# andi611/ZeroSpeech-TTS-without-T

Hardware: AMD Instinct MI355X
Metric: mel-frames/sec (train_ae, seg_len=128, enc_size=1024) (higher is better)
Workload: dtype bf16; 1 GPU; train_ae english hps seg_len=128 enc_size=1024 emb_size=1024 n_speakers=102 F=513, batch=256/GPU, dropout+Gumbel on, fwd+bwd+clip+Adam; global_batch=256, parallelism=dp1

## Files before the change

include/zs_amd.h:

```cpp
#ifndef ZS_AMD_H
#define ZS_AMD_H
#include <stddef.h>
#include <stdint.h>

#ifdef __cplusplus
extern "C" {
#endif

#define ZS_ABI_VERSION 1

enum { ZS_F32 = 0, ZS_BF16 = 1 };
enum { ZS_OK = 0, ZS_EINVAL = -1, ZS_ELAUNCH = -2, ZS_EWORKSPACE = -3 };
enum { ZS_PAD_ZERO = 0, ZS_PAD_REFLECT = 1 };
enum { ZS_ACT_NONE = 0, ZS_ACT_LRELU = 1, ZS_ACT_SIGMOID = 2, ZS_ACT_TANH = 3 };
enum { ZS_STORE_ROWS = 0, ZS_STORE_SPLIT2 = 1 };
enum { ZS_RES_NONE = 0, ZS_RES_IDENTITY = 1, ZS_RES_AVGPOOL2 = 2, ZS_RES_UPSAMPLE2 = 3 };

int zs_abi_version(void);
const char* zs_last_error(void);
int zs_set_option(const char* key, int value);

typedef struct {
  int32_t dtype;
  const void* A; int64_t lda; int64_t a_batch_stride;
// ... 80 lines not shown
  const void* x; int64_t ldx;
  void* out; int64_t ldo;
  void* out2; int64_t ldo2; const float* vec2; int64_t vec2_ld; int32_t vec2_cols; const int64_t* idx;
  float* mean; float* rstd;
  int32_t B, T, C; float eps;
  float drop_p; uint64_t seed; uint32_t stream_id; const uint8_t* mask; int64_t mask_ld;
  int32_t res_mode; const void* res; int64_t ldres; int32_t T_res; int32_t res_pad_mode;
  const uint64_t* seed_ptr;
  const int32_t* lengths; const int32_t* res_lengths;
  int32_t stats_given;
} ZsInstNormFwd;
int zs_instnorm_fwd(const ZsInstNormFwd* p, void* stream);

typedef struct {
  int32_t dtype;
  const void* dout; int64_t ldd;
  const void* x; int64_t ldx;
  const float* mean; const float* rstd;
  void* dz; int64_t ldz;
  int32_t B, T, C;
  float drop_p; uint64_t seed; uint32_t stream_id; const uint8_t* mask; int64_t mask_ld;
  float slope;
  const uint64_t* seed_ptr;
} ZsInstNormBwd;
int zs_instnorm_bwd(const ZsInstNormBwd* p, void* stream);

typedef struct {
  int32_t dtype;
  const void* gp; int64_t ldg; int32_t pad_left, pad_right, pad_mode;
  int32_t B, T, C;
  float* emb_sum; int64_t emb_ld; int32_t emb_cols;
  int32_t res_mode; const void* res; int64_t ldres;
  const void* dact_src; int64_t dact_ld; float slope;
  void* out; int64_t ldo; int32_t unshuffle;
} ZsGradCombine;
int zs_grad_combine(const ZsGradCombine* p, void* stream);
int zs_norm_decomposition(int32_t kernel, int32_t dtype, int32_t T, int32_t C);

typedef struct {
  const float* emb_sum; int64_t emb_ld; const int64_t* idx; int32_t B;
  float* demb; int64_t demb_ld; int32_t n_rows, C; int32_t accumulate;
} ZsEmbScatter;
int zs_emb_scatter(const ZsEmbScatter* p, void* stream);

typedef struct {
  int32_t dtype;
  const void* logits; int64_t ld; int32_t logits_f32;
  const float* noise; int32_t noise_kind; uint64_t seed;
  int64_t rows; int32_t E; float tau;
  void* bits; int64_t ld_bits; int32_t bits_fill_cols;
  float* bits_f32;
  float* y0;
  const uint64_t* seed_ptr;
} ZsMbvFwd;
int zs_mbv_fwd(const ZsMbvFwd* p, void* stream);
typedef struct {
  int32_t dtype;
  const void* dbits; int64_t ld_dbits;
  const float* y0; int64_t rows; int32_t E; float tau;
  void* dlogits; int64_t ld; int32_t fill_cols;
} ZsMbvBwd;
int zs_mbv_bwd(const ZsMbvBwd* p, void* stream);

enum { ZS_ENC_ONE_HOT = 0, ZS_ENC_BINARY = 1, ZS_ENC_CONTINUES = 2 };
typedef struct {
  int32_t dtype; int32_t mode;
// ... 295 lines not shown
```

zerospeech-tts-without-t_amd/_lib.py:

```python
import ctypes
import os
import re

_PKG = os.path.dirname(os.path.abspath(__file__))
_ROOT = os.path.dirname(_PKG)
HEADER = os.path.join(_ROOT, 'include', 'zs_amd.h')
_SAN = os.environ.get('ZS_SANITIZE', '').strip()
LIB_PATH = os.environ.get('ZS_LIB_PATH') or os.path.join(_PKG, 'libzs_amd.%s.so' % _SAN if _SAN else 'libzs_amd.so')

_CTYPES = {
    'int32_t': ctypes.c_int32, 'int64_t': ctypes.c_int64, 'uint32_t': ctypes.c_uint32, 'uint64_t': ctypes.c_uint64,
    'float': ctypes.c_float, 'double': ctypes.c_double, 'size_t': ctypes.c_size_t, 'int': ctypes.c_int,
}


def _strip_comments(text):
    return re.sub(r'/\*.*?\*/', ' ', text, flags=re.S)


def parse_header(path=HEADER):
    text = _strip_comments(open(path).read())
    structs = {}
    for body, name in re.findall(r'typedef\s+struct\s*\{(.*?)\}\s*(\w+)\s*;', text, flags=re.S):
        fields = []
# ... 142 lines not shown
        self._outer = (_PACK, _VEC)
        _PACK, _VEC = [], []
        return self

    def __exit__(self, et, ev, tb):
        global _PACK, _VEC
        jobs, vjobs = _PACK, _VEC
        _PACK, _VEC = self._outer
        if et is None and jobs:
            S = STRUCTS['ZsPackWeight']
            arr = (S * len(jobs))(*jobs)
            fn = lib().zs_pack_weight_batch
            fn.argtypes = [ctypes.c_void_p, ctypes.c_int32, ctypes.c_int32, ctypes.c_void_p]
            check(fn(ctypes.addressof(arr), len(jobs), 0, self.stream), 'zs_pack_weight_batch')
        if et is None and vjobs:
            S = STRUCTS['ZsVecCopy']
            arr = (S * len(vjobs))(*vjobs)
            fn = lib().zs_copy_vec_batch
            fn.argtypes = [ctypes.c_void_p, ctypes.c_int32, ctypes.c_void_p]
            check(fn(ctypes.addressof(arr), len(vjobs), self.stream), 'zs_copy_vec_batch')
        return False


def call(fname, sname, stream, **kw):
    try:
        s = STRUCTS[sname](**{k: v for k, v in kw.items() if v is not None})
    except TypeError as e:
        raise KeyError('%s: %s' % (sname, e))
    if _PACK is not None and fname == 'zs_pack_weight':
        _PACK.append(s)
        return s
    fn = _FN.get(fname)
    if fn is None:
        fn = getattr(lib(), fname)
        fn.argtypes = [ctypes.c_void_p, ctypes.c_void_p]
        _FN[fname] = fn
    rc = fn(ctypes.addressof(s), stream)
    if rc != 0:
        check(rc, fname)
    return s
```

zerospeech-tts-without-t_amd/csrc/zs_elem.hip:

```cpp
#include <string.h>

#include "zs_common.h"

namespace {

constexpr int NTE = 256;

template <typename T> __device__ __forceinline__ float ldT(const void* p, int64_t i) { return Elem<T>::ld((const T*)p + i); }
template <typename T> __device__ __forceinline__ void stT(void* p, int64_t i, float v) { Elem<T>::st((T*)p + i, v); }

template <typename T>
__device__ __forceinline__ void pack_weight_body(const ZsPackWeight& p, int64_t first, int64_t step) {
  const int64_t total = (int64_t)p.n_rows * p.n_cols;
  for (int64_t i = first; i < total; i += step) {
    const int row = (int)(i / p.n_cols);
    const int k = (int)(i - (int64_t)row * p.n_cols);
    const int tap = k / p.inner_pad, inner = k - tap * p.inner_pad;
    int n, ci;
    if (p.transpose == 0) { n = row; ci = inner; } else { n = inner; ci = row; }
    float v = 0.f;
    if (n < p.Cout && ci < p.Cin && tap < p.taps) {
      const int half = p.Cout >> 1;
      const int co = p.row_perm ? p.row_perm[n] : (p.co_split2 ? (n < half ? 2 * n : 2 * (n - half) + 1) : n);
      v = p.W[(int64_t)co * p.so + (int64_t)ci * p.si + (int64_t)tap * p.sj];
// ... 177 lines not shown
__global__ __launch_bounds__(128) void emb_scatter_kernel(const ZsEmbScatter p) {
  __shared__ int list[128];
  __shared__ int wcount[2];
  const int tid = threadIdx.x, lane = tid & 63, wave = tid >> 6;
  const int c = blockIdx.x * 128 + tid;
  const int r = blockIdx.y;
  float s = 0.f;
  for (int b0 = 0; b0 < p.B; b0 += 128) {
    const int b = b0 + tid;
    const bool hit = b < p.B && p.idx[b] == (int64_t)r;
    const unsigned long long m = __ballot(hit);
    if (lane == 0) wcount[wave] = __popcll(m);
    __syncthreads();
    const int n0 = wcount[0], n = n0 + wcount[1];
    if (hit) list[(wave ? n0 : 0) + __popcll(m & ((1ull << lane) - 1ull))] = b;
    __syncthreads();
    if (c < p.C)
      for (int i = 0; i < n; ++i) s += p.emb_sum[(int64_t)list[i] * p.emb_ld + c];
    __syncthreads();
  }
  if (c >= p.C) return;
  float* d = p.demb + (int64_t)r * p.demb_ld + c;
  *d = p.accumulate ? (*d + s) : s;
}

template <typename T>
__global__ void mbv_fwd_kernel(const ZsMbvFwd p) {
  const int64_t total = p.rows * p.bits_fill_cols;
  const uint64_t seed = p.seed + (p.seed_ptr ? *p.seed_ptr : 0ull);
  for (int64_t i = (int64_t)blockIdx.x * blockDim.x + threadIdx.x; i < total; i += (int64_t)gridDim.x * blockDim.x) {
    const int64_t r = i / p.bits_fill_cols;
    const int e = (int)(i - r * p.bits_fill_cols);
    float bit = 0.f;
    if (e < p.E) {
      float l0, l1;
      if (p.logits_f32) { l0 = ((const float*)p.logits)[r * p.ld + 2 * e]; l1 = ((const float*)p.logits)[r * p.ld + 2 * e + 1]; }
      else { l0 = ldT<T>(p.logits, r * p.ld + 2 * e); l1 = ldT<T>(p.logits, r * p.ld + 2 * e + 1); }
      const int64_t ni = (r * p.E + e) * 2;
      float g0, g1;
      if (p.noise_kind == 0) { g0 = p.noise[ni]; g1 = p.noise[ni + 1]; }
      else {
        float u0, u1;
        if (p.noise_kind == 1) { u0 = p.noise[ni]; u1 = p.noise[ni + 1]; }
        else { u0 = zs_uniform(seed, 0x6d627600u, (uint64_t)ni); u1 = zs_uniform(seed, 0x6d627600u, (uint64_t)ni + 1); }
        g0 = -logf(-logf(u0 + 1e-20f) + 1e-20f);
        g1 = -logf(-logf(u1 + 1e-20f) + 1e-20f);
// ... 319 lines not shown
  ZS_DISPATCH(p->dtype, add_rowvec_kernel, dim3(nblocks((int64_t)p->B * p->T * p->fill_cols, 4096)), dim3(NTE), stream, *p);
  return zs_check_launch("zs_add_rowvec");
}

extern "C" int zs_rows_reverse(const ZsRowsReverse* p, void* stream) {
  ZS_REQUIRE(p && p->x && p->B > 0 && p->T > 0 && p->cols > 0 && p->col0 >= 0 && p->ld >= (int64_t)p->col0 + p->cols, "zs_rows_reverse: bad args");
  ZS_REQUIRE(p->dtype == ZS_F32 || p->dtype == ZS_BF16, "zs_rows_reverse: bad dtype");
  const int es = p->dtype == ZS_F32 ? 4 : 2;
  ZS_REQUIRE((p->cols * es) % 4 == 0 && (p->col0 * es) % 4 == 0 && (p->ld * es) % 4 == 0 && (((uintptr_t)p->x) & 3) == 0,
             "zs_rows_reverse: the column block must be made of whole 4-byte words");
  if (p->T < 2) return ZS_OK;
  const int words = p->cols * es / 4;
  hipLaunchKernelGGL(rows_reverse_kernel, dim3(nblocks((int64_t)p->B * (p->T >> 1) * words, 4096)), dim3(NTE), 0, (hipStream_t)stream, *p, words,
                     (int64_t)p->ld * es, (int64_t)p->col0 * es);
  return zs_check_launch("zs_rows_reverse");
}

extern "C" int zs_emb_scatter(const ZsEmbScatter* p, void* stream) {
  ZS_REQUIRE(p && p->emb_sum && p->idx && p->demb && p->B > 0 && p->n_rows > 0 && p->C > 0, "zs_emb_scatter: bad args");
  hipLaunchKernelGGL(emb_scatter_kernel, dim3((p->C + 127) / 128, p->n_rows), dim3(128), 0, (hipStream_t)stream, *p);
  return zs_check_launch("zs_emb_scatter");
}

extern "C" int zs_mbv_fwd(const ZsMbvFwd* p, void* stream) {
  ZS_REQUIRE(p && p->logits && p->rows > 0 && p->E > 0 && p->tau > 0.f, "zs_mbv_fwd: bad args");
  ZS_REQUIRE(p->dtype == ZS_F32 || p->dtype == ZS_BF16, "zs_mbv_fwd: bad dtype");
  ZS_REQUIRE(p->noise_kind == 2 || p->noise, "zs_mbv_fwd: noise missing");
  ZS_REQUIRE(p->bits || p->bits_f32, "zs_mbv_fwd: no output");
  ZsMbvFwd q = *p;
  if (!q.bits || q.bits_fill_cols < q.E) q.bits_fill_cols = q.E;
  ZS_DISPATCH(p->dtype, mbv_fwd_kernel, dim3(nblocks(q.rows * q.bits_fill_cols)), dim3(NTE), stream, q);
  return zs_check_launch("zs_mbv_fwd");
}

extern "C" int zs_mbv_bwd(const ZsMbvBwd* p, void* stream) {
  ZS_REQUIRE(p && p->dbits && p->y0 && p->dlogits && p->rows > 0 && p->E > 0 && p->fill_cols >= 2 * p->E && p->fill_cols % 2 == 0,
             "zs_mbv_bwd: bad args");
  ZS_REQUIRE(p->dtype == ZS_F32 || p->dtype == ZS_BF16, "zs_mbv_bwd: bad dtype");
  ZS_DISPATCH(p->dtype, mbv_bwd_kernel, dim3(nblocks(p->rows * (p->fill_cols / 2))), dim3(NTE), stream, *p);
  return zs_check_launch("zs_mbv_bwd");
}

extern "C" int zs_l1_loss(const ZsL1Loss* p, void* stream) {
  ZS_REQUIRE(p && p->x_dec && p->x && p->partial && p->loss_out && p->rows > 0 && p->F > 0, "zs_l1_loss: bad args");
  ZS_REQUIRE(p->dtype == ZS_F32 || p->dtype == ZS_BF16, "zs_l1_loss: bad dtype");
  ZsL1Loss q = *p;
// ... 48 lines not shown
```

zerospeech-tts-without-t_amd/csrc/zs_norm.hip:

```cpp
#include <stdlib.h>

#include "zs_common.h"

namespace {

constexpr int RPT = 8;
struct Narrow { static constexpr int NTN = 256, CHUNK = 64, RG = 32; };
struct Wide8 { static constexpr int NTN = 256, CHUNK = 256, RG = 8; };
constexpr int RGN = 32;

template <typename S>
__device__ __forceinline__ void colreduce(const float (&pv)[RGN / S::RG][8], float (&out)[8], float* red, float* tot, int cg, int rg, int tid) {
  constexpr int CHUNK = S::CHUNK, RG = S::RG, NP = RGN / RG;
#pragma unroll
  for (int j = 0; j < NP; ++j)
#pragma unroll
    for (int k = 0; k < 8; ++k) red[(rg + RG * j) * CHUNK + cg * 8 + k] = pv[j][k];
  __syncthreads();
  for (int c = tid; c < CHUNK; c += S::NTN) {
    float s = 0.f;
#pragma unroll 8
    for (int r = 0; r < RGN; ++r) s += red[r * CHUNK + c];
    tot[c] = s;
  }
// ... 171 lines not shown
    if (cvalid && t < p.T) {
      const int64_t row = (int64_t)b * p.T + t;
      g[i].ld((const T*)p.dout + row * p.ldd + c0);
      xv[i].ld((const T*)p.x + row * p.ldx + c0);
    }
  }
#pragma unroll
  for (int i = 0; i < RPT; ++i) {
    const int t = rg + RG * i;
    if (cvalid && t < p.T) {
      const int64_t row = (int64_t)b * p.T + t;
      float gf[8], xf[8];
      g[i].cvt(gf); xv[i].cvt(xf);
#pragma unroll
      for (int k = 0; k < 8; ++k) {
        gf[k] *= keep_scale(p.mask, p.mask_ld, p.drop_p, seed, p.stream_id, row, c0 + k, p.C, inv_keep);
        const float xh = (xf[k] - mean[k]) * rstd[k];
        pg[i % NP][k] += gf[k]; pgx[i % NP][k] += gf[k] * xh;
      }
    }
  }
  colreduce<S>(pg, sg, red, tot, cg, rg, tid);
  colreduce<S>(pgx, sgx, red, tot, cg, rg, tid);
  if (!cvalid) return;
  const float invT = 1.f / (float)p.T;
#pragma unroll
  for (int i = 0; i < RPT; ++i) {
    const int t = rg + RG * i;
    if (t >= p.T) continue;
    const int64_t row = (int64_t)b * p.T + t;
    float o[8], gf[8], xf[8];
    g[i].cvt(gf); xv[i].cvt(xf);
#pragma unroll
    for (int k = 0; k < 8; ++k) {
      gf[k] *= keep_scale(p.mask, p.mask_ld, p.drop_p, seed, p.stream_id, row, c0 + k, p.C, inv_keep);
      const float xh = (xf[k] - mean[k]) * rstd[k];
      const float dx = rstd[k] * (gf[k] - sg[k] * invT - xh * (sgx[k] * invT));
      o[k] = dx * dlrelu_f(xf[k], p.slope);
    }
    store8<T>((T*)p.dz + row * p.ldz + c0, o);
  }
}

template <typename T, typename S>
__global__ __launch_bounds__(S::NTN) void grad_combine_kernel(const ZsGradCombine p) {
  constexpr int CHUNK = S::CHUNK, RG = S::RG, CGN = S::CHUNK / 8, NP = RGN / RG;
  __shared__ float red[RGN * CHUNK];
  __shared__ float tot[CHUNK];
  const int tid = threadIdx.x, cg = tid % CGN, rg = tid / CGN;
  const int b = blockIdx.y, c0 = blockIdx.x * CHUNK + cg * 8;
  const bool cvalid = c0 < p.C;
  const int Tp = p.T + p.pad_left + p.pad_right;
  const T* gp = (const T*)p.gp;
  float v[RPT][8];
  float ps[NP][8], s[8];
#pragma unroll
  for (int j = 0; j < NP; ++j)
#pragma unroll
    for (int k = 0; k < 8; ++k) ps[j][k] = 0.f;
#pragma unroll
  for (int i = 0; i < RPT; ++i) {
    const int t = rg + RG * i;
#pragma unroll
// ... 140 lines not shown
```

zerospeech-tts-without-t_amd/engine.py:

```python
import functools
import os
import torch

from . import _lib as L
from .layers import (Act, ConvLayer, GruLayer, cast_rows, colsum_ok, fork_side, grad_combine, instnorm_bwd, instnorm_fwd, join_side,
                     next_uid, rup)

LRELU = L.ZS_ACT_LRELU


def _half_up(t):
    return (t + 1) // 2


def _norm_stats(ctx, training, prefix, key, n):
    if not training:
        return None, None
    return ctx.f32(prefix + 'mean' + key, n), ctx.f32(prefix + 'rstd' + key, n)


def ragged_lengths(who, lengths, training, B, T, lo):
    if training:
        raise L.ZsError('%s: ragged batches are an inference feature' % who)
    l0 = torch.as_tensor(lengths, dtype=torch.int32).reshape(-1)
# ... 271 lines not shown
class DecoderEngine(object):
    def __init__(self, ctx, P, G, c_in, c_out, c_h, c_a, ns, seg_len, output_mask=False):
        self.ctx = ctx
        self.uid = next_uid()
        self.E, self.F, self.ch, self.n_spk = c_in, c_out, c_h, c_a
        self.ns = float(ns)
        self.pad_mode = L.ZS_PAD_REFLECT if seg_len >= 64 else L.ZS_PAD_ZERO
        self.out_act = L.ZS_ACT_TANH if output_mask else L.ZS_ACT_SIGMOID
        if c_h % 32:
            raise ValueError('Decoder c_h must be a multiple of 32 (got %d)' % c_h)
        mk = functools.partial(ConvLayer.from_params, ctx, P, G, pad_mode=self.pad_mode)
        self.input_emb = mk('input_emb')
        self.convs = [(mk('conv%d' % a, split2=True), mk('conv%d' % b)) for a, b in ((1, 2), (3, 4), (5, 6))]
        self.dense = [(mk('dense%d' % a), mk('dense%d' % b)) for a, b in ((1, 2), (3, 4))]
        self.gru = GruLayer(ctx, P, G, 'RNN.', name='dec%d' % self.uid)
        self.dense5 = mk('dense5')
        self.linear = mk('linear')
        self.emb = [P['emb%d.weight' % i] for i in range(1, 6)]
        self.gemb = [G['emb%d.weight' % i] for i in range(1, 6)]
        self.e_dense, self.e_rnn = 3, 4
        self.layers = [self.input_emb] + [l for p in self.convs for l in p] + [l for p in self.dense for l in p] + \
            [self.dense5, self.linear]
        self.tape = None

    def pack(self):
        with L.pack_batch(self.ctx.stream):
            for l in self.layers:
                l.pack()
            self.gru.pack()

    def forward(self, bits, cidx, training, lengths=None):
        c, ns, ch = self.ctx, self.ns, self.ch
        B, T0 = bits.B, bits.T
        Ls = [None] * 4
        if lengths is not None:
            l0 = ragged_lengths('DecoderEngine', lengths, training, B, T0, 2)
            ld = torch.stack([l0, 2 * l0, 4 * l0, 8 * l0]).to(c.device, non_blocking=True)
            Ls = [ld[i] for i in range(4)]
        tag = '_%d_%d_%d' % (self.uid, B, T0)
        st = c.stream
        emb = self.emb
        tp = {'B': B, 'T0': T0, 'training': training, 'cidx': cidx, 'bits': bits, 'blocks': [], 'dense': []}
        x = c.act('d_x0' + tag, B, T0, ch)
        xe = c.act('d_xe0' + tag, B, T0, ch)
        self.input_emb.fwd(bits, out=x, out2=xe, vec2=emb[0], idx=cidx)
        T = T0
        for i, (la, lb) in enumerate(self.convs):
            ya = c.act('d_ya%d' % i + tag, B, T, 2 * ch) if training else None
            s = c.act('d_s%d' % i + tag, B, 2 * T, ch)
            la.fwd(xe, out=ya, act=LRELU, slope=ns, out2=s, vec2=emb[i], idx=cidx, store_mode2=L.ZS_STORE_SPLIT2, lengths=Ls[i])
            yb = c.act('d_yb%d' % i + tag, B, 2 * T, ch)
            lb.fwd(s, out=yb, act=LRELU, slope=ns, lengths=Ls[i + 1])
            xn = c.act('d_x%d' % (i + 1) + tag, B, 2 * T, ch)
            xen = c.act('d_xe%d' % (i + 1) + tag, B, 2 * T, ch)
            nxt = emb[i + 1] if i < 2 else emb[3]
            stt = _norm_stats(c, training, 'd_', '%d_c%d_%d_%d' % (self.uid, i, B, 2 * T), B * yb.ld)
            instnorm_fwd(c, yb, xn, *stt, self.pad_mode, res_mode=L.ZS_RES_UPSAMPLE2, res=x, lengths=Ls[i + 1], out2=xen, vec2=nxt,
                         idx=cidx)
            tp['blocks'].append((x, xe, ya, s, yb, stt, T))
            x, xe, T = xn, xen, 2 * T
        return self._fwd_dense(tp, x, xe, cidx, T, tag, B, training, Ls[3])

    def _fwd_dense(self, tp, x, xe, cidx, T, tag, B, training, lengths):
        c, ns, ch, emb = self.ctx, self.ns, self.ch, self.emb
        ed, er = self.e_dense, self.e_rnn
        cat3 = c.act('d_cat3' + tag, B, T, 3 * ch)
        for j, (la, lb) in enumerate(self.dense):
            y1 = c.act('d_y1%d' % j + tag, B, T, ch)
            y1e = c.act('d_y1e%d' % j + tag, B, T, ch)
            la.fwd(xe, out=y1, act=LRELU, slope=ns, out2=y1e, vec2=emb[ed], idx=cidx)
            y2 = c.act('d_y2%d' % j + tag, B, T, ch)
            lb.fwd(y1e, out=y2, act=LRELU, slope=ns)
            xn = c.act('d_dx%d' % j + tag, B, T, ch) if j == 0 else Act(cat3.t, B, T, ch, cat3.ld, 0, ch)
            xen = c.act('d_dxe%d' % j + tag, B, T, ch)
            stt = _norm_stats(c, training, 'd_', '%d_d%d_%d_%d' % (self.uid, j, B, T), B * y2.ld)
            instnorm_fwd(c, y2, xn, *stt, self.pad_mode, res_mode=L.ZS_RES_IDENTITY, res=x, lengths=lengths, out2=xen,
                         vec2=(emb[ed] if j == 0 else emb[er]), idx=cidx)
            tp['dense'].append((x, xe, y1, y1e, y2, stt))
            x, xe = xn, xen
        H = ch // 2
        gi = c.act('d_gi' + tag, B, T, 6 * H)
        gates = c.raw('d_gates' + tag, B * T * 8 * H, c.tdt) if training else None
        self.gru.fwd(xe, cat3, ch, gi, gates, bcast=(emb[er], cidx, 2 * ch), lengths=lengths)
        h5 = c.act('d_h5' + tag, B, T, ch)
        self.dense5.fwd(cat3, out=h5, act=LRELU, slope=ns)
        return self._fwd_tail(c, tp, h5, cat3, gates, xe, T, tag, B)

    def _fwd_tail(self, c, tp, h5, cat3, gates, xe, T, tag, B):
        xdec = c.act('d_xdec' + tag, B, T, self.F, dtype=torch.float32)
        self.linear.fwd(h5, out=xdec, act=self.out_act, out_f32=True)
        tp.update(cat3=cat3, gates=gates, gru_in=xe, h5=h5, T=T)
        self.tape = tp
        return xdec

    def backward(self, dlogit, need_dbits=True):
        self.backward_head(dlogit)
        return self.backward_convs(need_dbits)

    def backward_head(self, dlogit):
        c, ns, ch, tp = self.ctx, self.ns, self.ch, self.tape
        assert tp is not None and tp['training']
        B, T0, T = tp['B'], tp['T0'], tp['T']
        tag = '_%d_%d_%d' % (self.uid, B, T0)
        cat3, h5 = tp['cat3'], tp['h5']
        H = ch // 2
        ed, er = self.e_dense, self.e_rnn
        self._embsum = c.f32('d_embsum' + tag, 6 * B * ch)
        self._embsum.zero_()
        self.linear.wgrad(dlogit, h5)
        dz5 = c.act('d_dz5' + tag, B, T, ch)
        fuse = colsum_ok(T) and os.environ.get('ZS_FUSE_COLSUM', '1') == '1'
        esum = lambda k: L.ptr(self._embsum, k * B * ch)
        slot = lambda k, col0=0: (esum(k), ch, col0)
        thin5 = fuse and ch % 128 == 0 and os.environ.get('ZS_THIN_EMB5', '1') == '1'
        self.linear.dgrad(dlogit, T, dz5, dact_src=h5, slope=ns, colsum=(slot(5) if thin5 else None), colsum_post=True)
        self.dense5.wgrad(dz5, cat3)
        dcat3 = c.act('d_dcat3' + tag, B, T, 3 * ch)
        if thin5:
            self.dense5.dgrad(dz5, T, dcat3, n_cols=2 * ch)
            s32 = Act(self._embsum, B, 1, ch, ch, 5 * B * ch)
            sT = c.act('d_s5' + tag, B, 1, ch)
            cast_rows(c, s32.ptr(), ch, sT)
            slot4 = Act(self._embsum, B, 1, ch, ch, er * B * ch)
            self.dense5.dgrad(sT, 1, slot4, add_src=slot4, out_f32=True, add_f32=True, n_cols=ch, n_off=2 * ch)
        elif fuse:
            self.dense5.dgrad(dz5, T, dcat3, colsum=slot(er, 2 * ch), out_cols=2 * ch)
        else:
            self.dense5.dgrad(dz5, T, dcat3)
            grad_combine(c, dcat3.sub(2 * ch, ch), T, 0, 0, self.pad_mode, ch, None, ns, emb_sum=esum(er))
        dgi = c.act('d_dgi' + tag, B, T, 6 * H)
        dgh = c.act('d_dgh' + tag, B, T, 6 * H)
        gp = c.act('d_gpA' + tag, B, T + 2, ch)
        gpv = Act(gp.t, B, T, ch, gp.ld)
        dx = c.act('d_dxA' + tag, B, T, ch)
        if fuse:
            self.gru.bwd(dcat3, ch, cat3, ch, tp['gates'], tp['gru_in'], dgi, dgh, dx, add_src=dcat3.sub(0, ch), colsum=slot(er))
        else:
            self.gru.bwd(dcat3, ch, cat3, ch, tp['gates'], tp['gru_in'], dgi, dgh, gpv)
            grad_combine(c, gpv, T, 0, 0, self.pad_mode, ch, dx, ns, emb_sum=esum(er), res_mode=L.ZS_RES_IDENTITY, res=dcat3.sub(0, ch))
        for j in (1, 0):
            la, lb = self.dense[j]
            xin, xe, y1, y1e, y2, stt = tp['dense'][j]
            dz2 = c.act('d_dz2%d' % j + tag, B, T, ch)
            instnorm_bwd(c, dx, y2, *stt, dz2, ns)
            lb.wgrad(dz2, y1e)
            dz1 = c.act('d_dz1%d' % j + tag, B, T, ch)
            if fuse:
                lb.dgrad(dz2, T, dz1, dact_src=y1, slope=ns, colsum=slot(ed))
            else:
                lb.dgrad(dz2, T, gpv)
                grad_combine(c, gpv, T, 0, 0, self.pad_mode, ch, dz1, ns, emb_sum=esum(ed), dact=y1)
            la.wgrad(dz1, xe)
            dn = c.act('d_dxD%d' % j + tag, B, T, ch)
            if fuse:
                la.dgrad(dz1, T, dn, add_src=dx, colsum=slot(ed))
            else:
                la.dgrad(dz1, T, gpv)
                grad_combine(c, gpv, T, 0, 0, self.pad_mode, ch, dn, ns, emb_sum=esum(ed), res_mode=L.ZS_RES_IDENTITY, res=dx)
            dx = dn
        self._bw = (dx, gp, tag)

    def backward_convs(self, need_dbits=True):
        c, ns, ch, tp = self.ctx, self.ns, self.ch, self.tape
        dx, gp, tag = self._bw
        B, T0 = tp['B'], tp['T0']
        for i in (2, 1, 0):
            la, lb = self.convs[i]
            xin, xe, ya, s, yb, stt, Ti = tp['blocks'][i]
# ... 29 lines not shown

class PatcherEngine(DecoderEngine):

    def __init__(self, ctx, P, G, c_in, c_out, c_h, c_a, ns):
        self.ctx = ctx
        self.uid = next_uid()
        self.E, self.F, self.ch, self.n_spk = c_in, c_out, c_h, c_a
        self.ns = float(ns)
        self.pad_mode = L.ZS_PAD_ZERO
        self.out_act = L.ZS_ACT_SIGMOID
        if c_h % 32:
            raise ValueError('Spectrogram_Patcher c_h must be a multiple of 32 (got %d)' % c_h)
        mk = functools.partial(ConvLayer.from_params, ctx, P, G, pad_mode=self.pad_mode)
        self.input_layer = mk('input_layer')
        self.dense = [(mk('dense%d' % a), mk('dense%d' % b)) for a, b in ((1, 2), (3, 4))]
        self.gru = GruLayer(ctx, P, G, 'RNN.', name='sp%d' % self.uid)
        self.dense5 = mk('dense5')
        self.linear = mk('linear')
        self.emb = [P['emb1.weight'], P['emb2.weight']]
        self.gemb = [G['emb1.weight'], G['emb2.weight']]
        self.e_dense, self.e_rnn = 0, 1
        self.layers = [self.input_layer] + [l for p in self.dense for l in p] + [self.dense5, self.linear]
        self.tape = None

    def forward(self, xd, cidx, training, lengths=None):
        c, ch = self.ctx, self.ch
        B, T = xd.B, xd.T
        ln = None
        if lengths is not None:
            ln = ragged_lengths('PatcherEngine', lengths, training, B, T, 1).to(c.device, non_blocking=True)
        tag = '_%d_%d_%d' % (self.uid, B, T)
        xin = c.act('p_xin' + tag, B, T, self.E)
        cast_rows(c, xd.ptr(), xd.ld, xin)
        tp = {'B': B, 'T0': T, 'training': training, 'cidx': cidx, 'xin': xin, 'dense': []}
        x = c.act('d_x0' + tag, B, T, ch)
        xe = c.act('d_xe0' + tag, B, T, ch)
        self.input_layer.fwd(xin, out=x, out2=xe, vec2=self.emb[0], idx=cidx)
        return self._fwd_dense(tp, x, xe, cidx, T, tag, B, training, ln)

    def backward(self, dlogit, need_dbits=False):
        if need_dbits:
            raise L.ZsError('PatcherEngine: the gradient w.r.t. the input spectrogram is not computed')
        self.backward_head(dlogit)
        dx, _, _ = self._bw
        c, tp, B, ch = self.ctx, self.tape, self.tape['B'], self.ch
        for k in range(2):
# ... 86 lines not shown
```

zerospeech-tts-without-t_amd/layers.py:

```python
import ctypes
import os

import torch

from . import _lib as L


def colsum_ok(T):
    return T > 0 and 128 % T == 0


def rup(x, m):
    return (x + m - 1) // m * m


DTYPES = {'fp32': (L.ZS_F32, torch.float32), 'bf16': (L.ZS_BF16, torch.bfloat16)}
SLACK = 512
EPS_IN = 1e-5


class Act(object):
    __slots__ = ('t', 'B', 'T', 'C', 'ld', 'off', 'cols')

    def __init__(self, t, B, T, C, ld, off=0, cols=None):
# ... 198 lines not shown
            ev = dict(common, taps=ne, sj=2 * self.sj)
            od = dict(common, taps=no, sj=2 * self.sj, W=L.ptr(self.w, self.sj))
            L.call('zs_pack_weight', 'ZsPackWeight', c.stream, transpose=1, inner_pad=self.cout_pad, dst=L.ptr(self.wd),
                   ldw=self.ldw_d, n_rows=self.n_pad_d, n_cols=ne * self.cout_pad, **ev)
            L.call('zs_pack_weight', 'ZsPackWeight', c.stream, transpose=1, inner_pad=self.cout_pad, dst=L.ptr(self.wd),
                   ldw=self.ldw_d, n_rows=self.n_pad_d, n_cols=no * self.cout_pad, col_offset=ne * self.cout_pad, **od)
        else:
            L.call('zs_pack_weight', 'ZsPackWeight', c.stream, transpose=1, inner_pad=self.cout_pad, dst=L.ptr(self.wd),
                   ldw=self.ldw_d, n_rows=self.n_pad_d, n_cols=self.ldw_d, **common)
        if self.bias_p is not None:
            h = self.Cout // 2
            L.vec_copy(self.bias_p[:h], self.b, c.stream, src_stride=2)
            L.vec_copy(self.bias_p[h:], self.b[1:], c.stream, src_stride=2)

    def bias_ptr(self):
        if self.b is None:
            return None
        return L.ptr(self.bias_p if self.bias_p is not None else self.b)

    def t_out(self, T_in):
        return (T_in + self.pad_l + self.pad_r - self.k) // self.stride + 1

    def fwd(self, A, out=None, act=L.ZS_ACT_NONE, slope=0.0, out_f32=False, out_cols=None, store_mode=L.ZS_STORE_ROWS,
            out2=None, vec2=None, idx=None, store_mode2=L.ZS_STORE_ROWS, out2_cols=None, pre_vec=None, bias=True, lengths=None):
        c = self.ctx
        T_out = self.t_out(A.T)
        kw = dict(dtype=c.dt, A=A.ptr(), lda=A.ld, a_batch_stride=A.T * A.ld, B=A.B, T_in=A.T, T_out=T_out, taps=self.k,
                  stride=self.stride, pad_left=self.pad_l, pad_mode=self.pad_mode, gather=0, cin_pad=self.cin_pad,
                  W=L.ptr(self.wf), ldw=self.ldw, N=self.Cout, n_pad=self.n_pad, bias=(self.bias_ptr() if bias else None), act=act,
                  slope=slope, groups=1)
        if pre_vec is not None:
            kw.update(pre_vec=L.ptr(pre_vec), pre_vec_ld=pre_vec.shape[1], vec_idx=L.ptr(idx))
        if lengths is not None and self.k > 1:
            kw.update(lengths=L.ptr(lengths), pad_right=self.pad_r)
        if out is not None:
            kw.update(out=out.ptr(), ldc=out.ld, out_f32=int(out_f32), store_mode=store_mode,
                      out_cols=out_cols if out_cols is not None else (min(out.cols, rup(self.Cout, 32)) if store_mode == L.ZS_STORE_ROWS else self.Cout // 2))
        if out2 is not None:
            kw.update(out2=out2.ptr(), ldc2=out2.ld, store_mode2=store_mode2,
                      out2_cols=out2_cols if out2_cols is not None else (min(out2.cols, rup(self.Cout, 32)) if store_mode2 == L.ZS_STORE_ROWS else self.Cout // 2))
            if vec2 is not None:
                kw.update(vec2=L.ptr(vec2), vec2_ld=vec2.shape[1], vec_idx=L.ptr(idx))
        L.call('zs_gemm_conv', 'ZsGemmConv', c.stream, **kw)
        return T_out

    def dgrad(self, dY, T_x, out, dact_src=None, slope=0.0, add_src=None, out_f32=False, add_f32=False, colsum=None, out_cols=None,
              n_cols=None, n_off=0, colsum_post=False):
        c = self.ctx
        Tp = T_x + self.pad_l + self.pad_r
        if self.parity:
            if dact_src is not None or add_src is not None or colsum is not None or n_cols is not None or n_off:
                raise ValueError('stride-2 dgrad: dact_src, add_src, colsum, n_cols and n_off are not supported')
            return self._dgrad_parity(dY, Tp, out, out_f32, out_cols)
        N, n_pad = self.Cin, self.n_pad_d
        if n_cols is not None and (n_cols < self.Cin or n_off):
            N = n_cols
            n_pad = rup(n_cols, 256) if n_off + rup(n_cols, 256) <= self.n_pad_d else rup(n_cols, 128)
            if n_off + n_pad > self.n_pad_d:
                raise ValueError('dgrad: channel block [%d, %d) does not fit the packed weight (%d rows)' % (n_off, n_off + n_cols, self.n_pad_d))
        kw = dict(dtype=c.dt, A=dY.ptr(), lda=dY.ld, a_batch_stride=dY.T * dY.ld, B=dY.B, T_in=dY.T, T_out=Tp, taps=self.k,
                  stride=self.stride, pad_left=0, pad_mode=L.ZS_PAD_ZERO, gather=1, cin_pad=self.cout_pad,
                  W=L.ptr(self.wd, n_off * self.ldw_d), ldw=self.ldw_d, N=N, n_pad=n_pad, act=L.ZS_ACT_NONE, slope=slope,
                  out=out.ptr(), ldc=out.ld, out_cols=(out_cols if out_cols is not None else min(out.cols, rup(N, 32))),
                  store_mode=L.ZS_STORE_ROWS, groups=1, out_f32=int(out_f32))
        if dact_src is not None:
            kw.update(dact_src=dact_src.ptr(), dact_ld=dact_src.ld)
        if add_src is not None:
            kw.update(add_src=add_src.ptr(), add_ld=add_src.ld, add_f32=int(add_f32))
        if colsum is not None:
            kw.update(colsum=colsum[0], colsum_ld=colsum[1], colsum_col0=colsum[2], colsum_post=int(colsum_post))
        L.call('zs_gemm_conv', 'ZsGemmConv', c.stream, **kw)
        return Tp

    def _dgrad_parity(self, dY, Tp, out, out_f32, out_cols):
        c = self.ctx
        Te = Tp + (Tp & 1)
        if out.T != Te:
            raise ValueError('stride-2 dgrad: the output needs %d rows per sample (padded domain %d rounded up to even), got %d' % (Te, Tp, out.T))
        ne = (self.k + 1) // 2
        for par, taps in ((0, ne), (1, self.k // 2)):
            kw = dict(dtype=c.dt, A=dY.ptr(), lda=dY.ld, a_batch_stride=dY.T * dY.ld, B=dY.B, T_in=dY.T, T_out=Te // 2, taps=taps,
                      stride=1, pad_left=0, pad_mode=L.ZS_PAD_ZERO, gather=1, cin_pad=self.cout_pad,
                      W=L.ptr(self.wd, par * ne * self.cout_pad), ldw=self.ldw_d, N=self.Cin, n_pad=self.n_pad_d, act=L.ZS_ACT_NONE,
                      out=out.ptr(par * out.ld), ldc=2 * out.ld, out_cols=(out_cols if out_cols is not None else min(out.cols, rup(self.Cin, 32))),
                      store_mode=L.ZS_STORE_ROWS, groups=1, out_f32=int(out_f32))
            L.call('zs_gemm_conv', 'ZsGemmConv', c.stream, **kw)
        return Tp

    def wgrad(self, dY, X, accumulate=False, bias=True):
        c = self.ctx
        es = c.es
        y_cols = min(dY.cols, rup(self.Cout, 16 // es))
        x_cols = min(X.cols, rup(self.Cin, 16 // es))
        kw = dict(dtype=c.dt, dY=dY.ptr(), ldy=dY.ld, y_cols=y_cols, X=X.ptr(), ldx=X.ld, x_batch_stride=X.T * X.ld,
                  x_cols=x_cols, B=X.B, T_in=X.T, T_out=dY.T, taps=self.k, stride=self.stride, pad_left=self.pad_l,
                  pad_mode=self.pad_mode, Cout=self.Cout, Cin=self.Cin, dW=L.ptr(self.gw), so=self.so, si=self.si, sj=self.sj,
                  db=(L.ptr(self.gb) if bias else None), co_split2=int(self.split2), accumulate=int(accumulate), splits=0)
        wgrad_call(c, kw, self.sid)


class Conv2dLayer(object):

    def __init__(self, ctx, weight, bias, gweight, gbias, stride=2, pad_mode=L.ZS_PAD_REFLECT, name='', dgrad_only=False):
        self.ctx, self.name = ctx, name
        self.w, self.b, self.gw, self.gb = weight, bias, gweight, gbias
        self.Cout, self.Cin, self.k = weight.shape[0], weight.shape[1], weight.shape[2]
        if weight.dim() != 4 or weight.shape[3] != self.k or stride not in (1, 2):
            raise ValueError('Conv2dLayer: square kernels, stride 1 or 2')
        self.stride, self.pad_mode, self.pad = stride, pad_mode, self.k // 2
        self.taps = self.k * self.k
        kc = ctx.kc
        self.cin_pad, self.cout_pad = rup(self.Cin, kc), rup(self.Cout, kc)
        self.ldw, self.n_pad, self.n_pad_d = self.taps * self.cin_pad, rup(self.Cout, 128), rup(self.Cin, 128)
        dev, tdt = ctx.device, ctx.tdt
        self.wf = None if dgrad_only else torch.zeros(self.n_pad * self.ldw + SLACK, dtype=tdt, device=dev)
        self.nt = [(self.k + 1) // 2, self.k // 2] if stride == 2 else [self.k]
        self.wd = {}
        for ph in range(len(self.nt)):
            for pw in range(len(self.nt)):
                ld = self.nt[ph] * self.nt[pw] * self.cout_pad
                self.wd[(ph, pw)] = (torch.zeros(self.n_pad_d * ld + SLACK, dtype=tdt, device=dev), ld)
# ... 95 lines not shown
        if any(w is not None for w in sd['ws']):
            torch.cuda.synchronize(ctx.device)
        size = int(need * 1.25) + 1024
        sd['ws'] = [torch.empty(size, dtype=torch.uint8, device=ctx.device) for _ in sd['streams']]
        ws = sd['ws'][i]
    ev = torch.cuda.Event()
    ev.record(torch.cuda.current_stream(ctx.device))
    sd['streams'][i].wait_event(ev)
    sd['used'] = True
    return sd['streams'][i].cuda_stream, ws


def wgrad_call(ctx, kw, sid=None):
    S = L.STRUCTS['ZsGemmWgrad']
    s = S()
    for k, v in kw.items():
        if v is not None:
            setattr(s, k, v)
    need = L.lib().zs_gemm_wgrad_workspace_bytes(ctypes.byref(s))
    stream, ws = side_launch(ctx, sid, need)
    s.workspace = ws.data_ptr()
    s.workspace_bytes = ws.numel()
    L.check(L.lib().zs_gemm_wgrad(ctypes.byref(s), ctypes.c_void_p(stream)), 'zs_gemm_wgrad')


def instnorm_fwd(ctx, x, out, mean, rstd, pad_mode, res_mode=L.ZS_RES_NONE, res=None, lengths=None, res_lengths=None, p=0.0,
                 seed=0, stream_id=0, mask=None, seed_ptr=None, out2=None, vec2=None, idx=None):
    L.call('zs_instnorm_fwd', 'ZsInstNormFwd', ctx.stream, dtype=ctx.dt, x=x.ptr(), ldx=x.ld, out=out.ptr(), ldo=out.ld,
           out2=(out2.ptr() if out2 is not None else None), ldo2=(out2.ld if out2 is not None else 0), vec2=L.ptr(vec2),
           vec2_ld=(vec2.shape[1] if vec2 is not None else 0), vec2_cols=(vec2.shape[1] if vec2 is not None else 0), idx=L.ptr(idx),
           mean=L.ptr(mean), rstd=L.ptr(rstd), B=x.B, T=x.T, C=x.ld, eps=EPS_IN, drop_p=p, seed=seed, stream_id=stream_id,
           mask=L.ptr(mask), mask_ld=(mask.shape[-1] if mask is not None else 0), res_mode=res_mode,
           res=(res.ptr() if res is not None else None), ldres=(res.ld if res is not None else 0), T_res=(res.T if res is not None else 0),
           res_pad_mode=pad_mode, seed_ptr=seed_ptr, lengths=L.ptr(lengths), res_lengths=L.ptr(res_lengths))


def instnorm_bwd(ctx, dout, x, mean, rstd, dz, slope, p=0.0, seed=0, stream_id=0, mask=None, seed_ptr=None):
    L.call('zs_instnorm_bwd', 'ZsInstNormBwd', ctx.stream, dtype=ctx.dt, dout=dout.ptr(), ldd=dout.ld, x=x.ptr(), ldx=x.ld,
           mean=L.ptr(mean), rstd=L.ptr(rstd), dz=dz.ptr(), ldz=dz.ld, B=x.B, T=x.T, C=x.ld, drop_p=p, seed=seed, stream_id=stream_id,
           mask=L.ptr(mask), mask_ld=(mask.shape[-1] if mask is not None else 0), slope=slope, seed_ptr=seed_ptr)


def grad_combine(ctx, gp, T, pad_l, pad_r, pad_mode, C, out, slope, res_mode=L.ZS_RES_NONE, res=None, dact=None, emb_sum=None,
                 unshuffle=0):
    L.call('zs_grad_combine', 'ZsGradCombine', ctx.stream, dtype=ctx.dt, gp=gp.ptr(), ldg=gp.ld, pad_left=pad_l, pad_right=pad_r,
           pad_mode=pad_mode, B=gp.B, T=T, C=C, emb_sum=emb_sum, emb_ld=(C if emb_sum is not None else 0),
           emb_cols=(C if emb_sum is not None else 0), res_mode=res_mode, res=(res.ptr() if res is not None else None),
           ldres=(res.ld if res is not None else 0), dact_src=(dact.ptr() if dact is not None else None),
           dact_ld=(dact.ld if dact is not None else 0), slope=slope, out=(out.ptr() if out is not None else None),
           ldo=(out.ld if out is not None else 0), unshuffle=unshuffle)


def cast_rows(ctx, src, ld_src, dst, dst_f32=False, dst2=None, col_off2=0, act2=L.ZS_ACT_NONE, slope2=0.0):
    L.call('zs_cast_rows', 'ZsCastRows', ctx.stream, dtype=ctx.dt, src=src, ld_src=ld_src, src_f32=1, dst=dst.ptr(), ld_dst=dst.ld,
           dst_f32=int(dst_f32), col_off=0, rows=dst.rows, cols=dst.C, fill_cols=dst.ld, act=L.ZS_ACT_NONE,
           dst2=(dst2.ptr() if dst2 is not None else None), ld_dst2=(dst2.ld if dst2 is not None else 0), col_off2=col_off2,
           fill_cols2=(dst2.ld - col_off2 if dst2 is not None else 0), act2=act2, slope2=slope2)


class GruLayer(object):

    def __init__(self, ctx, P, G, prefix, name=''):
        self.ctx, self.name = ctx, name
# ... 115 lines not shown
```

Before: 3.085 million frames/s.

## Fold constant speaker-embedding columns into precomputed tables and per-sample weight gradients

In the decoder's dense layers, the speaker embedding added per sample and the embedding columns of dense5's input are constant across time. The change precomputes W·emb tables at pack time and adds them as a per-row pre-vector, which removes the materialized y1e tensor and shrinks dense5's K dimension to 2*ch. In backward, instnorm_bwd now also emits per-sample column sums of dz. A new small emb_wgrad kernel then computes the embedding part of the weight gradient as S^T·emb over the batch instead of over B*T rows. This trades a large GEMM slice for extra kernels, table repacking each step and some bf16 rounding emulation.

```diff
diff --git a/include/zs_amd.h b/include/zs_amd.h
--- a/include/zs_amd.h
+++ b/include/zs_amd.h
@@ -126,6 +126,7 @@
   float drop_p; uint64_t seed; uint32_t stream_id; const uint8_t* mask; int64_t mask_ld;
   float slope;
   const uint64_t* seed_ptr;
+  float* colsum;
 } ZsInstNormBwd;
 int zs_instnorm_bwd(const ZsInstNormBwd* p, void* stream);
 
@@ -146,6 +147,15 @@
   float* demb; int64_t demb_ld; int32_t n_rows, C; int32_t accumulate;
 } ZsEmbScatter;
 int zs_emb_scatter(const ZsEmbScatter* p, void* stream);
+
+typedef struct {
+  int32_t dtype;
+  const float* S; int64_t lds;
+  const float* emb; int64_t emb_ld; const int64_t* idx; int32_t n_rows;
+  int32_t B, Cout, Cin;
+  float* dW; int64_t ldw; int64_t col_off; int32_t accumulate;
+} ZsEmbWgrad;
+int zs_emb_wgrad(const ZsEmbWgrad* p, void* stream);
 
 typedef struct {
   int32_t dtype;
diff --git a/zerospeech-tts-without-t_amd/_lib.py b/zerospeech-tts-without-t_amd/_lib.py
--- a/zerospeech-tts-without-t_amd/_lib.py
+++ b/zerospeech-tts-without-t_amd/_lib.py
@@ -188,6 +188,15 @@
         return False
 
 
+def conv_path(s):
+    fn = lib().zs_gemm_conv_path
+    fn.argtypes = [ctypes.c_void_p]
+    rc = fn(ctypes.addressof(s))
+    if rc < 0:
+        check(rc, 'zs_gemm_conv_path')
+    return rc
+
+
 def call(fname, sname, stream, **kw):
     try:
         s = STRUCTS[sname](**{k: v for k, v in kw.items() if v is not None})
diff --git a/zerospeech-tts-without-t_amd/csrc/zs_elem.hip b/zerospeech-tts-without-t_amd/csrc/zs_elem.hip
--- a/zerospeech-tts-without-t_amd/csrc/zs_elem.hip
+++ b/zerospeech-tts-without-t_amd/csrc/zs_elem.hip
@@ -223,6 +223,61 @@
   if (c >= p.C) return;
   float* d = p.demb + (int64_t)r * p.demb_ld + c;
   *d = p.accumulate ? (*d + s) : s;
+}
+
+constexpr int EW_TB = 16;
+template <bool BF>
+__global__ __launch_bounds__(256) void emb_wgrad_kernel(const ZsEmbWgrad p) {
+  __shared__ float sS[EW_TB][64];
+  __shared__ float sE[EW_TB][64];
+  const int tid = threadIdx.x, tx = tid & 15, ty = tid >> 4;
+  const int ci0 = blockIdx.x * 64, co0 = blockIdx.y * 64;
+  float acc[4][4];
+#pragma unroll
+  for (int i = 0; i < 4; ++i)
+#pragma unroll
+    for (int j = 0; j < 4; ++j) acc[i][j] = 0.f;
+  for (int b0 = 0; b0 < p.B; b0 += EW_TB) {
+    for (int i = tid; i < EW_TB * 64; i += 256) {
+      const int r = i >> 6, c = i & 63, b = b0 + r;
+      float s = 0.f, e = 0.f;
+      if (b < p.B) {
+        const int64_t row = p.idx[b];
+        if (row >= 0 && row < p.n_rows) {
+          if (co0 + c < p.Cout) s = p.S[(int64_t)b * p.lds + co0 + c];
+          if (ci0 + c < p.Cin) {
+            e = p.emb[row * p.emb_ld + ci0 + c];
+            if (BF) e = bf2f(f2bf(e));
+          }
+        }
+      }
+      sS[r][c] = s; sE[r][c] = e;
+    }
+    __syncthreads();
+#pragma unroll
+    for (int r = 0; r < EW_TB; ++r) {
+      float sv[4], ev[4];
+#pragma unroll
+      for (int i = 0; i < 4; ++i) { sv[i] = sS[r][ty * 4 + i]; ev[i] = sE[r][tx * 4 + i]; }
+#pragma unroll
+      for (int i = 0; i < 4; ++i)
+#pragma unroll
+        for (int j = 0; j < 4; ++j) acc[i][j] = fmaf(sv[i], ev[j], acc[i][j]);
+    }
+    __syncthreads();
+  }
+#pragma unroll
+  for (int i = 0; i < 4; ++i) {
+    const int co = co0 + ty * 4 + i;
+    if (co >= p.Cout) continue;
+#pragma unroll
+    for (int j = 0; j < 4; ++j) {
+      const int ci = ci0 + tx * 4 + j;
+      if (ci >= p.Cin) continue;
+      float* d = p.dW + (int64_t)co * p.ldw + p.col_off + ci;
+      *d = p.accumulate ? (*d + acc[i][j]) : acc[i][j];
+    }
+  }
 }
 
 template <typename T>
@@ -588,6 +643,19 @@
   return zs_check_launch("zs_emb_scatter");
 }
 
+extern "C" int zs_emb_wgrad(const ZsEmbWgrad* p, void* stream) {
+  ZS_REQUIRE(p && p->S && p->emb && p->idx && p->dW, "zs_emb_wgrad: null operand");
+  ZS_REQUIRE(p->dtype == ZS_F32 || p->dtype == ZS_BF16, "zs_emb_wgrad: bad dtype");
+  ZS_REQUIRE(p->B > 0 && p->Cout > 0 && p->Cin > 0 && p->n_rows > 0 && p->lds >= p->Cout && p->emb_ld >= p->Cin && p->col_off >= 0 &&
+                 p->ldw >= p->col_off + p->Cin,
+             "zs_emb_wgrad: sizes (B %d, Cout %d, Cin %d, lds %lld, emb_ld %lld, ldw %lld, col_off %lld)", p->B, p->Cout, p->Cin,
+             (long long)p->lds, (long long)p->emb_ld, (long long)p->ldw, (long long)p->col_off);
+  const dim3 grid((p->Cin + 63) / 64, (p->Cout + 63) / 64);
+  if (p->dtype == ZS_BF16) hipLaunchKernelGGL(emb_wgrad_kernel<true>, grid, dim3(256), 0, (hipStream_t)stream, *p);
+  else hipLaunchKernelGGL(emb_wgrad_kernel<false>, grid, dim3(256), 0, (hipStream_t)stream, *p);
+  return zs_check_launch("zs_emb_wgrad");
+}
+
 extern "C" int zs_mbv_fwd(const ZsMbvFwd* p, void* stream) {
   ZS_REQUIRE(p && p->logits && p->rows > 0 && p->E > 0 && p->tau > 0.f, "zs_mbv_fwd: bad args");
   ZS_REQUIRE(p->dtype == ZS_F32 || p->dtype == ZS_BF16, "zs_mbv_fwd: bad dtype");
diff --git a/zerospeech-tts-without-t_amd/csrc/zs_norm.hip b/zerospeech-tts-without-t_amd/csrc/zs_norm.hip
--- a/zerospeech-tts-without-t_amd/csrc/zs_norm.hip
+++ b/zerospeech-tts-without-t_amd/csrc/zs_norm.hip
@@ -217,12 +217,17 @@
   }
   colreduce<S>(pg, sg, red, tot, cg, rg, tid);
   colreduce<S>(pgx, sgx, red, tot, cg, rg, tid);
-  if (!cvalid) return;
+  const bool want_sum = p.colsum != nullptr;
+  if (!cvalid && !want_sum) return;
   const float invT = 1.f / (float)p.T;
 #pragma unroll
-  for (int i = 0; i < RPT; ++i) {
-    const int t = rg + RG * i;
-    if (t >= p.T) continue;
+  for (int j = 0; j < NP; ++j)
+#pragma unroll
+    for (int k = 0; k < 8; ++k) pg[j][k] = 0.f;
+#pragma unroll
+  for (int i = 0; i < RPT; ++i) {
+    const int t = rg + RG * i;
+    if (!cvalid || t >= p.T) continue;
     const int64_t row = (int64_t)b * p.T + t;
     float o[8], gf[8], xf[8];
     g[i].cvt(gf); xv[i].cvt(xf);
@@ -234,6 +239,17 @@
       o[k] = dx * dlrelu_f(xf[k], p.slope);
     }
     store8<T>((T*)p.dz + row * p.ldz + c0, o);
+    if (want_sum) {
+#pragma unroll
+      for (int k = 0; k < 8; ++k) pg[i % NP][k] += (sizeof(T) == 2) ? bf2f(f2bf(o[k])) : o[k];
+    }
+  }
+  if (want_sum) {
+    colreduce<S>(pg, sg, red, tot, cg, rg, tid);
+    if (cvalid && rg == 0) {
+#pragma unroll
+      for (int k = 0; k < 8; ++k) p.colsum[(int64_t)b * p.C + c0 + k] = sg[k];
+    }
   }
 }
 
diff --git a/zerospeech-tts-without-t_amd/engine.py b/zerospeech-tts-without-t_amd/engine.py
--- a/zerospeech-tts-without-t_amd/engine.py
+++ b/zerospeech-tts-without-t_amd/engine.py
@@ -317,12 +317,37 @@
         self.layers = [self.input_emb] + [l for p in self.convs for l in p] + [l for p in self.dense for l in p] + \
             [self.dense5, self.linear]
         self.tape = None
+        self._init_thin()
+
+    def _init_thin(self):
+        self.thin_knob = self.ch % 128 == 0 and os.environ.get('ZS_THIN_EMB', '1') == '1'
+        self._tab = None
+
+    def thin_emb(self, T):
+        return self.thin_knob and colsum_ok(T) and os.environ.get('ZS_FUSE_COLSUM', '1') == '1'
+
+    def _pack_tables(self):
+        c, ch = self.ctx, self.ch
+        e_d, e_r = self.emb[self.e_dense], self.emb[self.e_rnn]
+        n = e_d.shape[0]
+        if self._tab is None:
+            acts = [c.act('d_tab%d_%d' % (i, self.uid), 1, n, ch, dtype=torch.float32) for i in range(3)]
+            self._tab = (acts, [a.t[:n * a.ld].view(n, a.ld) for a in acts],
+                         [c.act('d_tabA%d_%d' % (i, self.uid), 1, n, ch) for i in range(2)])
+        acts, _, embA = self._tab
+        cast_rows(c, L.ptr(e_d), e_d.shape[1], embA[0])
+        cast_rows(c, L.ptr(e_r), e_r.shape[1], embA[1])
+        for j in range(2):
+            self.dense[j][1].fwd(embA[0], out=acts[j], out_f32=True, bias=False)
+        self.dense5.fwd(embA[1], out=acts[2], out_f32=True, bias=False, k_cols=ch, k_off=2 * ch)
 
     def pack(self):
         with L.pack_batch(self.ctx.stream):
             for l in self.layers:
                 l.pack()
             self.gru.pack()
+        if self.thin_knob:
+            self._pack_tables()
 
     def forward(self, bits, cidx, training, lengths=None):
         c, ns, ch = self.ctx, self.ns, self.ch
@@ -360,12 +385,19 @@
         c, ns, ch, emb = self.ctx, self.ns, self.ch, self.emb
         ed, er = self.e_dense, self.e_rnn
         cat3 = c.act('d_cat3' + tag, B, T, 3 * ch)
+        thin = tp['thin'] = self.thin_emb(T)
+        tabs = self._tab[1] if thin else None
         for j, (la, lb) in enumerate(self.dense):
             y1 = c.act('d_y1%d' % j + tag, B, T, ch)
-            y1e = c.act('d_y1e%d' % j + tag, B, T, ch)
-            la.fwd(xe, out=y1, act=LRELU, slope=ns, out2=y1e, vec2=emb[ed], idx=cidx)
             y2 = c.act('d_y2%d' % j + tag, B, T, ch)
-            lb.fwd(y1e, out=y2, act=LRELU, slope=ns)
+            if thin:
+                y1e = None
+                la.fwd(xe, out=y1, act=LRELU, slope=ns)
+                lb.fwd(y1, out=y2, act=LRELU, slope=ns, pre_vec=tabs[j], idx=cidx)
+            else:
+                y1e = c.act('d_y1e%d' % j + tag, B, T, ch)
+                la.fwd(xe, out=y1, act=LRELU, slope=ns, out2=y1e, vec2=emb[ed], idx=cidx)
+                lb.fwd(y1e, out=y2, act=LRELU, slope=ns)
             xn = c.act('d_dx%d' % j + tag, B, T, ch) if j == 0 else Act(cat3.t, B, T, ch, cat3.ld, 0, ch)
             xen = c.act('d_dxe%d' % j + tag, B, T, ch)
             stt = _norm_stats(c, training, 'd_', '%d_d%d_%d_%d' % (self.uid, j, B, T), B * y2.ld)
@@ -376,9 +408,13 @@
         H = ch // 2
         gi = c.act('d_gi' + tag, B, T, 6 * H)
         gates = c.raw('d_gates' + tag, B * T * 8 * H, c.tdt) if training else None
-        self.gru.fwd(xe, cat3, ch, gi, gates, bcast=(emb[er], cidx, 2 * ch), lengths=lengths)
+        bcast = None if (thin and not training) else (emb[er], cidx, 2 * ch)
+        self.gru.fwd(xe, cat3, ch, gi, gates, bcast=bcast, lengths=lengths)
         h5 = c.act('d_h5' + tag, B, T, ch)
-        self.dense5.fwd(cat3, out=h5, act=LRELU, slope=ns)
+        if thin:
+            self.dense5.fwd(cat3, out=h5, act=LRELU, slope=ns, k_cols=2 * ch, pre_vec=tabs[2], idx=cidx)
+        else:
+            self.dense5.fwd(cat3, out=h5, act=LRELU, slope=ns)
         return self._fwd_tail(c, tp, h5, cat3, gates, xe, T, tag, B)
 
     def _fwd_tail(self, c, tp, h5, cat3, gates, xe, T, tag, B):
@@ -408,8 +444,22 @@
         esum = lambda k: L.ptr(self._embsum, k * B * ch)
         slot = lambda k, col0=0: (esum(k), ch, col0)
         thin5 = fuse and ch % 128 == 0 and os.environ.get('ZS_THIN_EMB5', '1') == '1'
-        self.linear.dgrad(dlogit, T, dz5, dact_src=h5, slope=ns, colsum=(slot(5) if thin5 else None), colsum_post=True)
-        self.dense5.wgrad(dz5, cat3)
+        thin = tp['thin']
+        if thin and not fuse:
+            raise L.ZsError('DecoderEngine: ZS_FUSE_COLSUM changed between the forward and the backward pass')
+        cidx = tp['cidx']
+        self.linear.dgrad(dlogit, T, dz5, dact_src=h5, slope=ns, colsum=(slot(5) if (thin5 or thin) else None), colsum_post=True)
+        if thin:
+            s5 = esum(5)
+            if c.dt != L.ZS_F32 and not (L.conv_path(self.linear.last_dgrad) >> 8) & 1:
+                s5w = c.f32('d_s5w' + tag, B * ch)
+                s5w.zero_()
+                s5 = L.ptr(s5w)
+                grad_combine(c, dz5, T, 0, 0, self.pad_mode, ch, None, ns, emb_sum=s5)
+            st5 = self.dense5.wgrad(dz5, cat3, cin=2 * ch)
+            self.dense5.wgrad_const(s5, self.emb[er], cidx, col_off=2 * ch, stream=st5)
+        else:
+            self.dense5.wgrad(dz5, cat3)
         dcat3 = c.act('d_dcat3' + tag, B, T, 3 * ch)
         if thin5:
             self.dense5.dgrad(dz5, T, dcat3, n_cols=2 * ch)
@@ -437,8 +487,14 @@
             la, lb = self.dense[j]
             xin, xe, y1, y1e, y2, stt = tp['dense'][j]
             dz2 = c.act('d_dz2%d' % j + tag, B, T, ch)
-            instnorm_bwd(c, dx, y2, *stt, dz2, ns)
-            lb.wgrad(dz2, y1e)
+            if thin:
+                s2 = c.f32('d_s2%d' % j + tag, B * y2.ld)
+                instnorm_bwd(c, dx, y2, *stt, dz2, ns, colsum=L.ptr(s2))
+                st2 = lb.wgrad(dz2, y1)
+                lb.wgrad_const(L.ptr(s2), self.emb[ed], cidx, accumulate=True, stream=st2)
+            else:
+                instnorm_bwd(c, dx, y2, *stt, dz2, ns)
+                lb.wgrad(dz2, y1e)
             dz1 = c.act('d_dz1%d' % j + tag, B, T, ch)
             if fuse:
                 lb.dgrad(dz2, T, dz1, dact_src=y1, slope=ns, colsum=slot(ed))
@@ -514,6 +570,7 @@
         self.e_dense, self.e_rnn = 0, 1
         self.layers = [self.input_layer] + [l for p in self.dense for l in p] + [self.dense5, self.linear]
         self.tape = None
+        self._init_thin()
 
     def forward(self, xd, cidx, training, lengths=None):
         c, ch = self.ctx, self.ch
diff --git a/zerospeech-tts-without-t_amd/layers.py b/zerospeech-tts-without-t_amd/layers.py
--- a/zerospeech-tts-without-t_amd/layers.py
+++ b/zerospeech-tts-without-t_amd/layers.py
@@ -244,12 +244,19 @@
         return (T_in + self.pad_l + self.pad_r - self.k) // self.stride + 1
 
     def fwd(self, A, out=None, act=L.ZS_ACT_NONE, slope=0.0, out_f32=False, out_cols=None, store_mode=L.ZS_STORE_ROWS,
-            out2=None, vec2=None, idx=None, store_mode2=L.ZS_STORE_ROWS, out2_cols=None, pre_vec=None, bias=True, lengths=None):
+            out2=None, vec2=None, idx=None, store_mode2=L.ZS_STORE_ROWS, out2_cols=None, pre_vec=None, bias=True, lengths=None,
+            k_cols=None, k_off=0):
         c = self.ctx
         T_out = self.t_out(A.T)
+        cin_pad, w_off = self.cin_pad, 0
+        if k_cols is not None:
+            if self.k != 1 or k_cols % c.kc or k_off % c.kc or k_off + k_cols > self.cin_pad:
+                raise ValueError('fwd: k_cols / k_off need a 1-tap layer and whole K chunks inside the operand (%d + %d of %d)' %
+                                 (k_off, k_cols, self.cin_pad))
+            cin_pad, w_off = k_cols, k_off
         kw = dict(dtype=c.dt, A=A.ptr(), lda=A.ld, a_batch_stride=A.T * A.ld, B=A.B, T_in=A.T, T_out=T_out, taps=self.k,
-                  stride=self.stride, pad_left=self.pad_l, pad_mode=self.pad_mode, gather=0, cin_pad=self.cin_pad,
-                  W=L.ptr(self.wf), ldw=self.ldw, N=self.Cout, n_pad=self.n_pad, bias=(self.bias_ptr() if bias else None), act=act,
+                  stride=self.stride, pad_left=self.pad_l, pad_mode=self.pad_mode, gather=0, cin_pad=cin_pad,
+                  W=L.ptr(self.wf, w_off), ldw=self.ldw, N=self.Cout, n_pad=self.n_pad, bias=(self.bias_ptr() if bias else None), act=act,
                   slope=slope, groups=1)
         if pre_vec is not None:
             kw.update(pre_vec=L.ptr(pre_vec), pre_vec_ld=pre_vec.shape[1], vec_idx=L.ptr(idx))
@@ -291,7 +298,7 @@
             kw.update(add_src=add_src.ptr(), add_ld=add_src.ld, add_f32=int(add_f32))
         if colsum is not None:
             kw.update(colsum=colsum[0], colsum_ld=colsum[1], colsum_col0=colsum[2], colsum_post=int(colsum_post))
-        L.call('zs_gemm_conv', 'ZsGemmConv', c.stream, **kw)
+        self.last_dgrad = L.call('zs_gemm_conv', 'ZsGemmConv', c.stream, **kw)
         return Tp
 
     def _dgrad_parity(self, dY, Tp, out, out_f32, out_cols):
@@ -309,16 +316,25 @@
             L.call('zs_gemm_conv', 'ZsGemmConv', c.stream, **kw)
         return Tp
 
-    def wgrad(self, dY, X, accumulate=False, bias=True):
+    def wgrad(self, dY, X, accumulate=False, bias=True, cin=None):
         c = self.ctx
         es = c.es
+        Cin = self.Cin if cin is None else cin
         y_cols = min(dY.cols, rup(self.Cout, 16 // es))
-        x_cols = min(X.cols, rup(self.Cin, 16 // es))
+        x_cols = min(X.cols, rup(Cin, 16 // es))
         kw = dict(dtype=c.dt, dY=dY.ptr(), ldy=dY.ld, y_cols=y_cols, X=X.ptr(), ldx=X.ld, x_batch_stride=X.T * X.ld,
                   x_cols=x_cols, B=X.B, T_in=X.T, T_out=dY.T, taps=self.k, stride=self.stride, pad_left=self.pad_l,
-                  pad_mode=self.pad_mode, Cout=self.Cout, Cin=self.Cin, dW=L.ptr(self.gw), so=self.so, si=self.si, sj=self.sj,
+                  pad_mode=self.pad_mode, Cout=self.Cout, Cin=Cin, dW=L.ptr(self.gw), so=self.so, si=self.si, sj=self.sj,
                   db=(L.ptr(self.gb) if bias else None), co_split2=int(self.split2), accumulate=int(accumulate), splits=0)
-        wgrad_call(c, kw, self.sid)
+        return wgrad_call(c, kw, self.sid)
+
+    def wgrad_const(self, S, emb, idx, col_off=0, accumulate=False, stream=None):
+        c = self.ctx
+        if self.k != 1:
+            raise ValueError('wgrad_const: 1-tap layers only')
+        L.call('zs_emb_wgrad', 'ZsEmbWgrad', (stream if stream is not None else c.stream), dtype=c.dt, S=S, lds=self.Cout, emb=L.ptr(emb),
+               emb_ld=emb.shape[1], idx=L.ptr(idx), n_rows=emb.shape[0], B=idx.numel(), Cout=self.Cout, Cin=emb.shape[1],
+               dW=L.ptr(self.gw), ldw=self.so, col_off=col_off * self.si, accumulate=int(accumulate))
 
 
 class Conv2dLayer(object):
@@ -460,6 +476,7 @@
     s.workspace = ws.data_ptr()
     s.workspace_bytes = ws.numel()
     L.check(L.lib().zs_gemm_wgrad(ctypes.byref(s), ctypes.c_void_p(stream)), 'zs_gemm_wgrad')
+    return stream
 
 
 def instnorm_fwd(ctx, x, out, mean, rstd, pad_mode, res_mode=L.ZS_RES_NONE, res=None, lengths=None, res_lengths=None, p=0.0,
@@ -473,10 +490,10 @@
            res_pad_mode=pad_mode, seed_ptr=seed_ptr, lengths=L.ptr(lengths), res_lengths=L.ptr(res_lengths))
 
 
-def instnorm_bwd(ctx, dout, x, mean, rstd, dz, slope, p=0.0, seed=0, stream_id=0, mask=None, seed_ptr=None):
+def instnorm_bwd(ctx, dout, x, mean, rstd, dz, slope, p=0.0, seed=0, stream_id=0, mask=None, seed_ptr=None, colsum=None):
     L.call('zs_instnorm_bwd', 'ZsInstNormBwd', ctx.stream, dtype=ctx.dt, dout=dout.ptr(), ldd=dout.ld, x=x.ptr(), ldx=x.ld,
            mean=L.ptr(mean), rstd=L.ptr(rstd), dz=dz.ptr(), ldz=dz.ld, B=x.B, T=x.T, C=x.ld, drop_p=p, seed=seed, stream_id=stream_id,
-           mask=L.ptr(mask), mask_ld=(mask.shape[-1] if mask is not None else 0), slope=slope, seed_ptr=seed_ptr)
+           mask=L.ptr(mask), mask_ld=(mask.shape[-1] if mask is not None else 0), slope=slope, seed_ptr=seed_ptr, colsum=colsum)
 
 
 def grad_combine(ctx, gp, T, pad_l, pad_r, pad_mode, C, out, slope, res_mode=L.ZS_RES_NONE, res=None, dact=None, emb_sum=None,
```

After: 3.073 million frames/s. Within noise of the previous version (-0.4%).
